# ruuda/robigo-luculenta

Hardware: AMD Instinct MI355X
Metric: Mrays/sec on built-in scene at 1920x1080 (higher is better)
Workload: dtype f32

## Files before the change

### robigo_luculenta_amd/csrc/rl_api.hip

```cpp
#include <hip/hip_runtime.h>
#include <sys/prctl.h>

#include <dlfcn.h>
#include <unistd.h>

#include <algorithm>
#include <chrono>
#include <condition_variable>
#include <cstdio>
#include <cstdlib>
#include <cstring>
#include <atomic>
#include <map>
#include <memory>
#include <mutex>
#include <new>
#include <string>
#include <thread>
#include <vector>

#include <rccl/rccl.h>

#include "../../include/robigo_luculenta.h"
#include "../../include/robigo_luculenta_debug.h"
// ... 174 lines not shown
    };
    return table[index];
}
size_t ring_t_bytes(const RlScene* scene) { return scene->lay.n_cluster_supers != 0u ? (size_t)(RL_TRACE_BLOCK / 64) * 512u : 0u; }
int stage_of(const RlScene* scene, int fetch, size_t scratch_bytes, size_t* bytes) {
    *bytes = 0;
    if (fetch != RL_FETCH_LDS) return RL_STAGE_NONE;
    const size_t all = (scene->staged_bytes + 511) & ~(size_t)511, tables = (scene->tables_bytes + 511) & ~(size_t)511;
    if (scene->lay.n_cluster_supers == 0u && all + scratch_bytes <= 160 * 1024) {
        *bytes = all;
        return RL_STAGE_ALL;
    }
    if (tables + scratch_bytes <= 160 * 1024) {
        *bytes = tables;
        return RL_STAGE_TABLES;
    }
    return RL_STAGE_NONE;
}

int fetch_check(int fetch) {
    if (fetch != RL_FETCH_LDS && fetch != RL_FETCH_GLOBAL) return fail(RL_E_INVALID, "unknown fetch mode");
    return RL_OK;
}
int path_range_check(uint64_t first_path, uint64_t n) {
    if (first_path + n < first_path || first_path + n == ~0ull) return fail(RL_E_INVALID, "path indices must stay below 2^64 - 1");
    return RL_OK;
}
int max_segments_resolve(uint32_t max_segments, uint32_t* resolved) {
    if (max_segments > RL_PATH_MAX_SEGMENTS_CAP) return fail(RL_E_INVALID, "max_segments exceeds RL_PATH_MAX_SEGMENTS_CAP = 65536");
    *resolved = max_segments == 0u ? RL_PATH_MAX_SEGMENTS : max_segments;
    return RL_OK;
}

int launch_trace(RlTraceUnit* u, const RlScene* scene, RlMappedPhoton* photons, RlPlotUnit* plot_unit, uint64_t seed,
                 uint32_t stream_id, uint64_t first_path, uint64_t n_paths) {
    if (n_paths == 0) return RL_OK;
    if (path_range_check(first_path, n_paths) != RL_OK) return RL_E_INVALID;
    float* plot = plot_unit ? plot_unit->xyz : nullptr;
    if (scene->device != u->device) return fail(RL_E_STATE, "scene and trace unit live on different devices");
    RlTraceJob job;
    job.width = u->width;
    job.height = u->height;
    job.aspect_ratio = (float)u->width / (float)u->height;
    job.stream = stream_id;
    job.seed = seed;
    job.first_path = first_path;
    job.n_paths = n_paths;
    job.grace_ticks = 0;
    job.reserved = 0;
    job.wm1 = (float)(int)u->width - 1.0f;
    job.hm1 = (float)(int)u->height - 1.0f;

    const size_t scratch_bytes = (RL_TRACE_BLOCK / 64) * sizeof(RlWaveScratch) + ring_t_bytes(scene);
    size_t blob_bytes = 0;
    const int stage = stage_of(scene, u->fetch, scratch_bytes, &blob_bytes);
    const bool fused = plot != nullptr;
    const bool cyl = scene->lay.prism_cylinders != 0u;
    auto kernel = trace_kernel_variant(stage, fused, false, cyl);
    const size_t dyn = scratch_bytes + blob_bytes;
    if (u->tuned_per_cu == 0 || u->tuned_dyn != dyn || u->tuned_kernel != (const void*)kernel) {
        RL_HIP(hipFuncSetAttribute((const void*)kernel, hipFuncAttributeMaxDynamicSharedMemorySize, 160 * 1024));
        int per_cu = 1;
        RL_HIP(hipOccupancyMaxActiveBlocksPerMultiprocessor(&per_cu, kernel, RL_TRACE_BLOCK, dyn));
        u->tuned_per_cu = per_cu < 1 ? 1 : per_cu;
        if (getenv("RL_DEBUG_LAUNCH")) fprintf(stderr, "rl: trace launch: %d workgroup(s) of %d threads per CU, %zu bytes of LDS each, stage %d\n", per_cu, RL_TRACE_BLOCK, dyn, stage);
        u->tuned_dyn = dyn;
        u->tuned_kernel = (const void*)kernel;
    }
    uint64_t blocks = (uint64_t)u->cu_count * (uint64_t)u->tuned_per_cu;
    const uint64_t needed = (n_paths + RL_TRACE_BLOCK - 1) / RL_TRACE_BLOCK;
// ... 2411 lines not shown
```

### robigo_luculenta_amd/csrc/rl_kernels.hip.h

```cpp
#pragma once
#include <hip/hip_runtime.h>

#include <cstddef>
#include <type_traits>

#include "rl_cie1931.h"
#include "rl_core.h"

#define RL_BLOCK 256
#ifndef RL_TRACE_BLOCK
#define RL_TRACE_BLOCK 1024
#endif
#ifndef RL_TRACE_WPS
#define RL_TRACE_WPS 4
#endif
#ifndef RL_TRACE_VGPRS
#define RL_TRACE_VGPRS (RL_TRACE_WPS == 4 ? 128 : 96)
#endif
#ifndef RL_TRACE_VGPRS_OPEN
#define RL_TRACE_VGPRS_OPEN (RL_TRACE_WPS == 4 ? 120 : 96)
#endif
#define RL_EMIT_MAX_AGE 8u
#define RL_CHUNK 256ull

// ... 158 lines not shown
    float lhs;
    asm("v_fma_f32 %0, %1, %2, %3" : "=v"(lhs) : "v"(x), "v"(y), "v"(cs));
    return lhs;
}
__device__ __forceinline__ bool rl_cull_pass(const RlCullRay& r, RlF4 b, float far) {
    const float dd = __builtin_fmaf(r.d.z, b.z, __builtin_fmaf(r.d.y, b.y, __builtin_fmaf(r.d.x, b.x, r.p)));
    const float cs = __builtin_fmaf(r.m.z, b.z, __builtin_fmaf(r.m.y, b.y, __builtin_fmaf(r.m.x, b.x, b.w)));
    const float x = __builtin_amdgcn_fmed3f(dd, 0.0f, far);
    return __builtin_fmaf(x, __builtin_fmaf(-2.0f, dd, x), cs) <= r.q;
}

__device__ __forceinline__ bool rl_cyl_pass(const RlCullRay& r, RlF4 c, RlF3 a) {
    const float cox = __builtin_fmaf(0.5f, r.m.x, c.x), coy = __builtin_fmaf(0.5f, r.m.y, c.y), coz = __builtin_fmaf(0.5f, r.m.z, c.z);
    const float crx = __builtin_fmaf(r.d.y, a.z, -(r.d.z * a.y)), cry = __builtin_fmaf(r.d.z, a.x, -(r.d.x * a.z)),
                crz = __builtin_fmaf(r.d.x, a.y, -(r.d.y * a.x));
    const float w = __builtin_fmaf(coz, crz, __builtin_fmaf(coy, cry, cox * crx));
    const float radius = __builtin_fmaf(4.0e-6f, fabsf(cox) + fabsf(coy) + fabsf(coz), c.w);
    const float cr2 = __builtin_fmaf(crz, crz, __builtin_fmaf(cry, cry, crx * crx));
    return !(w * w > radius * radius * cr2);
}

struct RlWaveScratch {
    unsigned long long key[64];
    uint32_t ring_a[128];
    uint32_t ring_b[128];
    uint32_t ring_s[128];
    float terms_d[64][4];
    float terms_m[64][4];
    float far[64];
    float stash[10][64];
    float emit[5][64];
};
static_assert(sizeof(RlWaveScratch) == 8192, "rl_scan_wave's ring addressing wants the wave's scratch 512-byte aligned");

typedef float RlV4 __attribute__((ext_vector_type(4)));
typedef __attribute__((address_space(3))) RlV4 RlLdsV4;
typedef __attribute__((address_space(3))) float RlLdsF;
template <bool PF = false>
__device__ __forceinline__ void rl_store_cull_ray(RlWaveScratch* ws, uint32_t lane, const RlCullRay& cr, float far) {
    ((RlLdsV4*)&ws->terms_d[0][0])[lane] = (RlV4){cr.d.x, cr.d.y, cr.d.z, cr.p};
    ((RlLdsV4*)&ws->terms_m[0][0])[lane] = (RlV4){cr.m.x, cr.m.y, cr.m.z, cr.q};
    ((RlLdsF*)&ws->far[0])[lane] = PF ? cr.len : far;
}
template <bool PF = false>
__device__ __forceinline__ void rl_fetch_cull_ray(RlWaveScratch* ws, uint32_t owner, RlCullRay& r, float& r_far) {
    const RlV4 a = ((const RlLdsV4*)&ws->terms_d[0][0])[owner], b = ((const RlLdsV4*)&ws->terms_m[0][0])[owner];
    r_far = ((const RlLdsF*)&ws->far[0])[owner];
    if (PF) r_far *= rl_u2f(((const RlLdsU32*)&ws->key[0])[2u * owner + 1u]);
    r.d = rl_f3(a.x, a.y, a.z);
    r.p = a.w;
    r.m = rl_f3(b.x, b.y, b.z);
    r.q = b.w;
    r.len = 0.0f;
}
__device__ __forceinline__ void rl_fetch_ray(RlWaveScratch* ws, uint32_t owner, RlF3 dir, RlF3& ro, RlF3& rd) {
    const RlV4 b = ((const RlLdsV4*)&ws->terms_m[0][0])[owner];
    rl_fetch3(owner, dir.x, dir.y, dir.z, rd.x, rd.y, rd.z);
    asm volatile("" : : "v"(b.w));
    ro = rl_f3(b.x * -0.5f, b.y * -0.5f, b.z * -0.5f);
}

struct RlOpenWg {
    uint32_t fin[RL_OPEN_CAP];
    uint32_t seg[RL_OPEN_CAP];
    uint32_t flushed_at;
    uint32_t poll[2];
    uint32_t pad;
};

template <bool CYL, bool SPLIT, bool UNROLL_S, bool HOIST_S, bool SPHERES_IN_LDS, bool TABLES_IN_LDS, bool SUPER, bool BOUNDED = false>
__device__ __forceinline__ RlHit rl_scan_wave(const RlSceneView& sv, const RlF4* cull, const RlF4* prism_cyl, uint32_t group_gc, uint32_t small_ordered, float sv_cull_cmax2,
                                              uint32_t n_cluster_groups, uint32_t n_prism_groups, uint32_t n_cluster_supers, uint32_t super_g, RlLdsU32* ring_t, RlF3 o, RlF3 dir,
                                              uint32_t idle_bit, RlWaveScratch* ws, uint32_t lane RL_TACC_PARAM, float t_bound = 1.0e12f) {
    constexpr bool PF = SUPER;
    RlLdsU64* keys = (RlLdsU64*)ws->key;
    RlLdsU32* ring_a = (RlLdsU32*)ws->ring_a;
    RlLdsU32* ring_b = (RlLdsU32*)ws->ring_b;
    RlLdsU32* ring_s = (RlLdsU32*)ws->ring_s;
    uint32_t a_lim = 64u, a_tail = 0, b_lim = 64u, b_tail = 0, s_lim = 64u, s_tail = 0;
    const uint32_t ws_addr = (uint32_t)(size_t)(RlLdsU32*)ws;
#define RL_RING_SLOT(RING, M, TAIL) \
    ((RlLdsU32*)(size_t)((ws_addr | (((rl_mbcnt(M) + (TAIL)) << 2) & 0x1fcu)) + (uint32_t)offsetof(RlWaveScratch, RING)))
#define RL_RING_PUSH(RING, COND, M, TAIL, ENTRY)                                                                        \
    {                                                                                                                   \
        uint32_t slot_;                                                                                                 \
                \
        asm volatile("s_mov_b64 exec, %6\n\ts_nop 0\n\tv_mbcnt_lo_u32_b32 %0, %1, 0\n\tv_mbcnt_hi_u32_b32 %0, %2, %0\n\t"         \
                     "v_add_lshl_u32 %0, %0, %3, 2\n\tv_and_or_b32 %0, %0, %4, %5\n\tds_write_b32 %0, %7 offset:%8\n\ts_mov_b64 exec, -1" \
                     : "=&v"(slot_)                                                                                     \
                     : "s"((uint32_t)(M)), "s"((uint32_t)((M) >> 32)), "s"(TAIL), "s"(ring_mask), "v"(ws_addr), "s"(M),  \
                       "v"(ENTRY), "n"(offsetof(RlWaveScratch, RING))                                                   \
                     : "memory");                                                                                       \
    }
#define RL_LE_PUSH(RING, LHS, RHS, TAIL, ENTRY)                                                                        \
    {                                                                                                                   \
        uint32_t slot_, n_;                                                                                             \
         \
        asm volatile("v_cmpx_le_f32_e32 vcc, %2, %3\n\ts_bcnt1_i32_b64 %1, vcc\n\ts_nop 0\n\t"                              \
                     "v_mbcnt_lo_u32_b32 %0, vcc_lo, 0\n\tv_mbcnt_hi_u32_b32 %0, vcc_hi, %0\n\t"                            \
                     "v_add_lshl_u32 %0, %0, %4, 2\n\tv_and_or_b32 %0, %0, %5, %6\n\tds_write_b32 %0, %7 offset:%8\n\t"     \
                     "s_mov_b64 exec, -1"                                                                               \
                     : "=&v"(slot_), "=&s"(n_)                                                                           \
                     : "v"(LHS), "v"(RHS), "s"(TAIL), "s"(ring_mask), "v"(ws_addr), "v"(ENTRY),                          \
// ... 91 lines not shown
            RL_FENCE;
            parab(b0, b1, b2);
            const RlF4 d0 = sv.planes[0], d1 = sv.planes[1];
            RL_FENCE;
            parab(c0, c1, c2);
            const RlF4 e0 = sv.planes[2], e1 = sv.planes[3];
            RL_FENCE;
            plane(d0, d1);
            const RlF4 f0 = sv.planes[4], f1 = sv.planes[5];
            RL_FENCE;
            plane(e0, e1);
            plane(f0, f1);
#undef RL_FENCE
        };
        if ((small_ordered & 2u) != 0u) six(std::integral_constant<bool, true>());
        else six(std::integral_constant<bool, false>());
    } else if ((small_ordered & 1u) != 0u) {
        RL_SMALL_PRIMITIVES(RL_NEARER_ORDERED, n_parabs, n_planes)
    } else {
        RL_SMALL_PRIMITIVES(rl_nearer, n_parabs, n_planes)
    }
#undef RL_NEARER_ORDERED
#undef RL_SMALL_PRIMITIVES
    keys[lane] = ((unsigned long long)rl_f2u(best.t) << 32) |
                 (unsigned long long)(best.obj == RL_HIT_NONE ? 0xffffffffu : (best.obj << 3));
    RL_T1(RL_ST_T_SMALL, t_small);
    if constexpr (BOUNDED) {
        if (best.obj != RL_HIT_NONE && best.t < t_bound) idle_bit = 0x80000000u;
        if (__builtin_amdgcn_ballot_w64(idle_bit == 0u) == 0) return best;
    }

    RlCullRay cr = rl_cull_ray(o, dir, sv_cull_cmax2, idle_bit != 0u);
    float far = best.t * cr.len;
    rl_store_cull_ray<PF>(ws, lane, cr, far);
#define RL_REFRESH_FAR()                                                                                \
    if (PF) {                                                                                           \
        far = rl_u2f(((const RlLdsU32*)keys)[2u * lane + 1u]) * cr.len;                                 \
         \
        if constexpr (BOUNDED) {                                                                        \
            if (rl_u2f(((const RlLdsU32*)keys)[2u * lane + 1u]) < t_bound) cr.q = -__builtin_inff();    \
        }                                                                                               \
    }

    auto process_spheres = [&](uint32_t count) {
        RL_STAT(RL_ST_B_ROUNDS, 1);
        RL_STAT(RL_ST_B_LANES, count);
        RL_T0(t_b);
        rl_wave_sync();
        const uint32_t e = ring_b[(b_lim - 64u + lane) & 127u];
        const uint32_t owner = e & 63u;
        const uint32_t pos = (SPHERES_IN_LDS || lane < count) ? e >> 6 : 0u;
        const RlF4 s = sph[pos];
        const float s_r2 = sv.sphere_r2[pos];
        const uint32_t s_obj = sv.sphere_obj[pos];
        RlF3 fo, fd;
        rl_fetch_ray(ws, owner, dir, fo, fd);
        asm volatile("" : : "v"(s.w));
        const float ox = fo.x, oy = fo.y, oz = fo.z, dx = fd.x, dy = fd.y, dz = fd.z;
        if (lane < count) {
            const float cox = s.x - ox, coy = s.y - oy, coz = s.z - oz;
            const float dd = dx * cox + dy * coy + dz * coz;
            const float c = (cox * cox + coy * coy + coz * coz) - s_r2;
            const float q = dd * dd - c;
            const float sq = rl_sqrtf(q, true);
            const float t1 = dd - sq;
            const float t2 = dd + sq;
            if ((q >= 0.0f) & (t1 > 0.0f) & (t1 < t2)) {
                __hip_atomic_fetch_min(keys + owner, ((unsigned long long)rl_f2u(t1) << 32) | (unsigned long long)(s_obj << 3),
                                       __ATOMIC_RELAXED, __HIP_MEMORY_SCOPE_WAVEFRONT);
            }
        }
        rl_wave_sync();
        RL_T1(RL_ST_T_B_ROUNDS, t_b);
    };

#define RL_SPHERE_REJECT(S, POS, OWNER, DISABLE_BIT, OX, OY, OZ, DX, DY, DZ)                        \
    {                                                                                               \
        const float cox = (S).x - (OX), coy = (S).y - (OY), coz = (S).z - (OZ);                     \
        const float dd = (DX) * cox + (DY) * coy + (DZ) * coz;                                      \
        const float c = (cox * cox + coy * coy + coz * coz) - (S).w;                                \
        const float q = dd * dd - c;                                                                \
        const bool cand = (int)(rl_f2u(q) | (rl_f2u(dd) - 1u) | (DISABLE_BIT)) >= 0;               \
        const uint64_t m = __builtin_amdgcn_ballot_w64(cand);                                       \
        if (m != 0) {                                                                               \
            RL_RING_PUSH(ring_b, cand, m, b_tail, ((POS) << 6) | (OWNER))               \
            b_tail += (uint32_t)__popcll(m);                                                        \
            if (RL_UNLIKELY(b_tail >= b_lim)) {                                                           \
                process_spheres(64u);                                                               \
                b_lim += 64u;                                                                      \
// ... 295 lines not shown
#undef RL_SPHERE_REJECT
    RL_T1(RL_ST_T_CLUSTER, t_cluster);
    RL_T0(t_tailflush);
    if (b_tail != b_lim - 64u) process_spheres(b_tail - (b_lim - 64u));
    b_lim = b_tail + 64u;
    RL_T1(RL_ST_T_TAIL, t_tailflush);
    RL_T0(t_prism);
    far = rl_u2f((uint32_t)(keys[lane] >> 32)) * cr.len;
    if (!PF) ((RlLdsF*)&ws->far[0])[lane] = far;
    if constexpr (BOUNDED) {
        const unsigned long long k_now = keys[lane];
        if (rl_u2f((uint32_t)(k_now >> 32)) < t_bound) idle_bit = 0x80000000u;
        if (__builtin_amdgcn_ballot_w64(idle_bit == 0u) == 0) {
            best.t = rl_u2f((uint32_t)(k_now >> 32));
            best.obj = (uint32_t)k_now == 0xffffffffu ? RL_HIT_NONE : (uint32_t)k_now >> 3;
            best.sub = (uint32_t)k_now == 0xffffffffu ? 0u : (uint32_t)k_now & 7u;
            return best;
        }
    }

    auto process_prisms = [&](uint32_t count) {
        RL_STAT(RL_ST_P_ROUNDS, 1);
        RL_STAT(RL_ST_P_LANES, count);
        RL_T0(t_p);
        rl_wave_sync();
        uint32_t e = ring_a[(a_lim - 64u + lane) & 127u];
        uint32_t owner = e & 63u;
        const uint32_t prism = e >> 6;
        const RlF4* pr = sv.prisms + __umul24((uint32_t)RL_PRISM_STRIDE, lane < count ? prism : 0u);
        constexpr bool PRE = HOIST_S && SPLIT;
        RlF4 pre_n = RlF4(), pre_off = RlF4();
        if (PRE) pre_n = pr[0], pre_off = pr[1];
        RlF3 ro, rd;
        rl_fetch_ray(ws, owner, dir, ro, rd);
        RlCand c;
        int status = rl_hex_prism_fast<HOIST_S && SPLIT, PRE>(pr, ro, rd, &c, pre_n, pre_off);
        if (lane >= count) status = RL_PRISM_MISS;
        if (__builtin_amdgcn_ballot_w64(status == RL_PRISM_UNSURE) != 0) {
            RL_STAT(RL_ST_P_SLOW, 1);
            c = rl_hex_prism(pr, ro, rd);
            status = ((lane < count) & (c.t >= 0.0f)) ? RL_PRISM_HIT : RL_PRISM_MISS;
            {
                asm volatile("" ::: "memory");
                const float keep_len = cr.len;
                rl_fetch_cull_ray<PF>(ws, lane, cr, far);
                cr.len = keep_len;
            }
            uint32_t again = a_lim - 64u;
            asm volatile("" : "+s"(again) : : "memory");
            e = ring_a[(again + lane) & 127u];
            owner = e & 63u;
            pr = sv.prisms + __umul24((uint32_t)RL_PRISM_STRIDE, lane < count ? (e >> 6) : 0u);
        }
        if (status == RL_PRISM_HIT) {
            const uint32_t obj = rl_f2u(pr[1].w);
            const unsigned long long k = ((unsigned long long)rl_f2u(c.t) << 32) | (unsigned long long)((obj << 3) | c.k);
            __hip_atomic_fetch_min(keys + owner, k, __ATOMIC_RELAXED, __HIP_MEMORY_SCOPE_WAVEFRONT);
        }
        rl_wave_sync();
        RL_T1(RL_ST_T_P_ROUNDS, t_p);
    };
    auto process_cylinders = [&](uint32_t count) {
        rl_wave_sync();
        const uint32_t e = ring_b[(b_lim - 64u + lane) & 127u];
        const uint32_t owner = e & 63u;
        const RlF4* cy = prism_cyl + 2u * (lane < count ? (e >> 6) : 0u);
        const RlF4 cy0 = cy[0], cy1 = cy[1];
// ... 171 lines not shown
#endif
    typedef __attribute__((address_space(3))) float RlLdsF32;
    RlLdsF32* stash = (RlLdsF32*)&ws->stash[0][0];

    uint64_t chunk_next = 0, chunk_end = 0;
    uint32_t stash_head = 0, stash_count = 0;
    uint64_t stash_path0 = 0;
    uint32_t stash_valid = 0;
    bool drained = false;
    bool active = false;
    uint64_t my_path = 0;
    uint32_t my_job = 0;
    uint32_t stash_job = 0;
    uint64_t stash_first = job.first_path;
    RlPath p;
    p.origin = rl_f3(0.0f, 0.0f, 0.0f);
    p.direction = rl_f3(0.0f, 0.0f, 0.0f);
    p.wavelength = 0.0f;
    p.intensity = 0.0f;
    p.continue_chance = 0.0f;
    p.sx = p.sy = 0.0f;
    p.ior = 1.0f;
    p.bounce = 0;
    uint32_t segments = 0, paths_done = 0;
    uint32_t known_local = 0;
    bool pend_me = false;
    bool pend_any = false;
    uint32_t emit_pend = 0;
    RlOpenWg* wgp = (RlOpenWg*)(scratch + RL_TRACE_BLOCK / 64);
    RlLdsU32* wg_fin = (RlLdsU32*)&wgp->fin[0];
    RlLdsU32* wg_seg = (RlLdsU32*)&wgp->seg[0];
    RlLdsU32* wg_flushed_at = (RlLdsU32*)&wgp->flushed_at;
    RlLdsU32* wg_poll = (RlLdsU32*)&wgp->poll[0];
    RlLdsF32* emit = (RlLdsF32*)&ws->emit[0][0];
    auto emit_put = [&](uint32_t row, uint32_t slot, float v) {
        emit[row * 64u + slot] = v;
    };
    auto emit_get = [&](uint32_t row, uint32_t slot) -> float {
        return emit[row * 64u + slot];
    };
    if (OPEN) {
        for (uint32_t i = threadIdx.x; i < sizeof(RlOpenWg) / 4; i += RL_TRACE_BLOCK) ((RlLdsU32*)wgp)[i] = 0;
        __syncthreads();
    }
    auto settle = [&]() {
        if (!pend_any && emit_pend == 0) return;
        asm volatile("s_waitcnt vmcnt(0) ; rl_settle: results acknowledged" ::: "memory");
        __builtin_amdgcn_fence(__ATOMIC_RELEASE, "workgroup");
        if (pend_me) __hip_atomic_fetch_add(wg_fin + my_job, 1u, __ATOMIC_RELAXED, __HIP_MEMORY_SCOPE_WORKGROUP);
        if (lane < emit_pend)
            __hip_atomic_fetch_add(wg_fin + (((RlLdsU32*)ws->ring_b)[lane] >> 24), 1u, __ATOMIC_RELAXED,
                                   __HIP_MEMORY_SCOPE_WORKGROUP);
        pend_me = false;
        pend_any = false;
        emit_pend = 0;
    };
    auto flush = [&](uint32_t gap) {
        const uint32_t now = (uint32_t)wall_clock64();
        uint32_t mine = gap == 0u ? 1u : 0u;
        if (lane == 0 && gap != 0u) {
            uint32_t at = *wg_flushed_at;
            if (now - at >= gap)
                mine = __hip_atomic_compare_exchange_strong(wg_flushed_at, &at, now | 1u, __ATOMIC_RELAXED, __ATOMIC_RELAXED,
                                                            __HIP_MEMORY_SCOPE_WORKGROUP) ? 1u : 0u;
        }
        if (__builtin_amdgcn_readfirstlane(mine) == 0u) return;
        for (uint32_t base_job = 0; base_job < known_local; base_job += 64u) {
// ... 6 lines not shown
            if (__builtin_amdgcn_ballot_w64((f | sg) != 0u) == 0) continue;
            if (sg != 0) __hip_atomic_fetch_add(&od->seg[jb], sg, __ATOMIC_RELAXED, __HIP_MEMORY_SCOPE_AGENT);
            __builtin_amdgcn_fence(__ATOMIC_RELEASE, "workgroup");
            if (f != 0) {
                const uint32_t before = __hip_atomic_fetch_add(&od->fin[jb], f, __ATOMIC_RELAXED, __HIP_MEMORY_SCOPE_AGENT);
                if (before + f == (uint32_t)od->jobs[jb].end) {
                    __hip_atomic_fetch_add(&od->completed, 1u, __ATOMIC_RELAXED, __HIP_MEMORY_SCOPE_AGENT);
                    const uint32_t total = __hip_atomic_load(&od->seg[jb], __ATOMIC_RELAXED, __HIP_MEMORY_SCOPE_AGENT);
                    __hip_atomic_store(&ctl->segs[jb], total, __ATOMIC_RELAXED, __HIP_MEMORY_SCOPE_SYSTEM);
                    __hip_atomic_store(&ctl->done[jb], 1u, __ATOMIC_RELEASE, __HIP_MEMORY_SCOPE_SYSTEM);
                }
            }
        }
    };
    uint32_t e_head = 0, e_tail = 0;
    uint32_t emit_age = 0;
#ifdef RL_STATS
    unsigned long long st[RL_ST_COUNT];
    for (int k = 0; k < RL_ST_COUNT; ++k) st[k] = 0;
#endif
    RL_T0(t_total);

    auto process_emitted = [&](uint32_t count) {
        RL_STAT(RL_ST_EMIT_BATCHES, 1);
        RL_STAT(RL_ST_EMIT_LANES, count);
        if (OPEN && emit_pend != 0) settle();
        rl_wave_sync();
        if (!FUSED) {
            uint32_t idx = 0, tagged = 0;
            float value = 0.0f;
            RlMappedPhoton* dst_base = photons;
            if (lane < count) {
                const uint32_t slot = (e_head + lane) & 63u;
                idx = rl_f2u(emit_get(0, slot));
                tagged = rl_f2u(emit_get(4, slot));
                if (OPEN) ((RlLdsU32*)ws->ring_b)[lane] = tagged;
                uint64_t first = job.first_path;
                if (OPEN) {
                    const RlJobEntry e = jobs[tagged >> 24];
                    first = e.first_path, dst_base = (RlMappedPhoton*)e.target;
                }
                const RlRngBlock b0 = rl_rng_block(job.seed, job.stream, first + idx, 0);
                RlMappedPhoton ph;
                ph.wavelength = rl_get_wavelength(b0.w[0]);
                ph.x = rl_get_bi_unit(b0.w[1]);
                ph.y = rl_get_bi_unit(b0.w[2]) / job.aspect_ratio;
                value = rl_emission(sv, emit_get(3, slot), ph.wavelength, OPEN ? (tagged & 0xffffffu) : tagged);
                ph.probability = value;
                if (OPEN) {
                    uint32_t* dst = (uint32_t*)&dst_base[idx];
                    __hip_atomic_store(dst + 0, rl_f2u(ph.x), __ATOMIC_RELAXED, __HIP_MEMORY_SCOPE_AGENT);
                    __hip_atomic_store(dst + 1, rl_f2u(ph.y), __ATOMIC_RELAXED, __HIP_MEMORY_SCOPE_AGENT);
                    __hip_atomic_store(dst + 2, rl_f2u(ph.probability), __ATOMIC_RELAXED, __HIP_MEMORY_SCOPE_AGENT);
                    __hip_atomic_store(dst + 3, rl_f2u(ph.wavelength), __ATOMIC_RELAXED, __HIP_MEMORY_SCOPE_AGENT);
                } else {
                    dst_base[idx] = ph;
                }
            }
        } else if (lane < count) {
            const uint32_t slot = (e_head + lane) & 63u;
            const float sx = emit_get(0, slot), sy = emit_get(1, slot), wavelength = emit_get(2, slot);
            const uint32_t tagged = rl_f2u(emit_get(4, slot));
            if (OPEN) ((RlLdsU32*)ws->ring_b)[lane] = tagged;
            float* target = plot;
            if (OPEN) target = (float*)jobs[tagged >> 24].target;
            const float value = rl_emission(sv, emit_get(3, slot), wavelength, OPEN ? (tagged & 0xffffffu) : tagged);
            if (value != 0.0f) {
                const RlF3 cie = rl_mul(rl_tristimulus(sv.cie, wavelength), value);
                uint32_t width = job.width, height = job.height;
                asm volatile("" : "+s"(width), "+s"(height));
                const RlSplat sp = rl_splat_weights(width, height, job.wm1, job.hm1, job.aspect_ratio, sx, sy);
#pragma unroll
                for (int k = 0; k < 4; ++k) {
                    float* px = target + 3ull * sp.idx[k];
                    unsafeAtomicAdd(px + 0, cie.x * sp.w[k]);
                    unsafeAtomicAdd(px + 1, cie.y * sp.w[k]);
                    unsafeAtomicAdd(px + 2, cie.z * sp.w[k]);
                }
            }
        }
        if (OPEN) emit_pend = count;
        rl_wave_sync();
    };

    for (;;) {
        if (OPEN) {
            settle();
            flush(3000u);
        }
        RL_T0(t_refill);
        auto refill = [&]() -> bool {
            if (drained) return false;
                uint32_t open_n = 0;
                if (OPEN) {
                    bool got = false;
                    for (;;) {
                        if (chunk_next < chunk_end) {
                            open_n = (uint32_t)jobs[stash_job].end;
                            got = true;
// ... 101 lines not shown
                    }
                    if (!got) return false;
                }
                if (!OPEN && chunk_next == chunk_end) {
                    const unsigned long long chunk =
                        job.n_paths >= (unsigned long long)gridDim.x * (RL_TRACE_BLOCK * 16ull) ? RL_CHUNK : 64ull;
                    unsigned long long b = 0;
                    if (lane == 0) b = atomicAdd(&queue[0], chunk);
                    const uint32_t lo = __builtin_amdgcn_readfirstlane((uint32_t)b);
                    const uint32_t hi = __builtin_amdgcn_readfirstlane((uint32_t)(b >> 32));
                    chunk_next = ((uint64_t)hi << 32) | lo;
                    chunk_end = chunk_next + chunk;
                }
                RL_STAT(RL_ST_REFILLS, 1);
                if (OPEN) stash_first = jobs[stash_job].first_path;
                const uint64_t limit = OPEN ? (uint64_t)open_n : job.n_paths;
                stash_path0 = stash_first + chunk_next;
                stash_valid = chunk_next >= limit ? 0u : (limit - chunk_next >= 64ull ? 64u : (uint32_t)(limit - chunk_next));
                chunk_next += 64;
                const bool valid = lane < stash_valid;
                const uint64_t path_index = stash_path0 + lane;
                RlPath fresh = p;
                RL_T0(t_cam);
                if (valid) rl_begin_path(sv, job.aspect_ratio, job.seed, job.stream, path_index, &fresh);
                RL_T1(RL_ST_T_CAMERA, t_cam);
                rl_wave_sync();
                stash[0 * 64 + lane] = fresh.origin.x;
                stash[1 * 64 + lane] = fresh.origin.y;
                stash[2 * 64 + lane] = fresh.origin.z;
                stash[3 * 64 + lane] = fresh.direction.x;
                stash[4 * 64 + lane] = fresh.direction.y;
                stash[5 * 64 + lane] = fresh.direction.z;
                stash[6 * 64 + lane] = fresh.wavelength;
                stash[7 * 64 + lane] = fresh.sx;
                stash[8 * 64 + lane] = fresh.sy;
                stash[9 * 64 + lane] = fresh.ior;
                rl_wave_sync();
                stash_head = 0;
                stash_count = 64;
                if (!OPEN && chunk_next >= job.n_paths) drained = true;
            return true;
        };
        auto hand_out = [&](const uint64_t need) -> bool {
            const uint32_t avail = stash_count - stash_head;
            const uint32_t rank = rl_mbcnt(need);
            const uint32_t slot = stash_head + rank;
            const bool take = !active & (rank < avail) & (slot < stash_valid);
            {
                const uint32_t sl = slot & 63u;
                const float s0 = stash[0 * 64 + sl], s1 = stash[1 * 64 + sl], s2 = stash[2 * 64 + sl], s3 = stash[3 * 64 + sl], s4 = stash[4 * 64 + sl];
                const float s5 = stash[5 * 64 + sl], s6 = stash[6 * 64 + sl], s7 = stash[7 * 64 + sl], s8 = stash[8 * 64 + sl], s9 = stash[9 * 64 + sl];
                my_path = take ? stash_path0 + slot : my_path;
                if (OPEN) my_job = take ? stash_job : my_job;
                p.origin = rl_f3(take ? s0 : p.origin.x, take ? s1 : p.origin.y, take ? s2 : p.origin.z);
                p.direction = rl_f3(take ? s3 : p.direction.x, take ? s4 : p.direction.y, take ? s5 : p.direction.z);
                p.wavelength = take ? s6 : p.wavelength;
                p.sx = take ? s7 : p.sx;
                p.sy = take ? s8 : p.sy;
                p.ior = take ? s9 : p.ior;
                p.intensity = take ? 1.0f : p.intensity;
                p.continue_chance = take ? 1.0f : p.continue_chance;
                p.bounce = take ? 0u : p.bounce;
                active = active | take;
            }
            const uint32_t wanted = (uint32_t)__popcll(need);
            stash_head += wanted < avail ? wanted : avail;
            return wanted <= avail;
        };
        {
            const uint64_t need = __builtin_amdgcn_ballot_w64(!active);
            if (need != 0) {
                bool served = false;
                if (RL_LIKELY(stash_count != stash_head)) served = hand_out(need);
                if (RL_UNLIKELY(!served)) {
                    if (refill()) hand_out(__builtin_amdgcn_ballot_w64(!active));
                }
            }
        }
        RL_T1(RL_ST_T_REFILL, t_refill);
        if (__builtin_amdgcn_ballot_w64(active) == 0) {
            if (!OPEN || drained) break;
            settle();
            if (e_tail != e_head) {
                process_emitted(e_tail - e_head);
                e_head = e_tail;
                settle();
            }
            flush(500u);
            for (int k = 0; k < 4; ++k) __builtin_amdgcn_s_sleep(127);
            continue;
        }
        constexpr bool FULL = !OPEN || (STAGE == RL_STAGE_ALL && (FUSED || !CYL));
        const RlHit hit = rl_scan_wave<CYL, FULL, STAGE != RL_STAGE_NONE && (!(FUSED && OPEN) || FULL), STAGE != RL_STAGE_NONE && (!(OPEN && (FUSED || STAGE == RL_STAGE_TABLES)) || FULL), STAGE == RL_STAGE_ALL, STAGE != RL_STAGE_NONE, STAGE != RL_STAGE_ALL>(sv, base + (lay.off_cull - tab0), CYL ? base + (lay.off_prism_cyl - tab0) : nullptr, lay.group_gc, lay.small_ordered, lay.cull_cmax2, lay.n_cluster_groups, lay.n_prism_groups,
                                       lay.n_cluster_supers, lay.super_g, ring_t, p.origin, p.direction, active ? 0u : 0x80000000u, ws, lane RL_TACC_ARG);
#ifdef RL_STATS
        {
            const uint32_t mk = (active && hit.obj != RL_HIT_NONE) ? rl_object_material(rl_f2u(sv.objects[hit.obj].w)) : 99u;
            const uint64_t m_act = __builtin_amdgcn_ballot_w64(active);
            const uint64_t m_void = __builtin_amdgcn_ballot_w64(active && hit.obj == RL_HIT_NONE);
            const uint64_t m_emit = __builtin_amdgcn_ballot_w64(mk == RL_MATERIAL_BLACK_BODY);
            const uint64_t m_grey = __builtin_amdgcn_ballot_w64(mk == RL_MATERIAL_DIFFUSE_GREY);
            const uint64_t m_col = __builtin_amdgcn_ballot_w64(mk == RL_MATERIAL_DIFFUSE_COLOURED);
            const uint64_t m_gls = __builtin_amdgcn_ballot_w64(mk == RL_MATERIAL_GLOSSY_MIRROR);
            const uint64_t m_glass = __builtin_amdgcn_ballot_w64(mk == RL_MATERIAL_SF10_GLASS);
            const uint64_t m_soap = __builtin_amdgcn_ballot_w64(mk == RL_MATERIAL_SOAP_BUBBLE);
            RL_STAT(RL_ST_ITER, 1);
            RL_STAT(RL_ST_SCAN_LANES, __popcll(m_act));
            RL_STAT(RL_ST_END_VOID, __popcll(m_void));
            RL_STAT(RL_ST_END_EMITTER, __popcll(m_emit));
            RL_STAT(RL_ST_SHADE_DIFFUSE, __popcll(m_grey | m_col | m_gls));
            RL_STAT(RL_ST_SHADE_GLASS, __popcll(m_glass));
            RL_STAT(RL_ST_SHADE_SOAP, __popcll(m_soap));
            RL_STAT(RL_ST_ANY_DIFFUSE, (m_grey | m_col | m_gls) != 0);
            RL_STAT(RL_ST_ANY_GLASS, m_glass != 0);
            RL_STAT(RL_ST_ANY_SOAP, m_soap != 0);
            RL_STAT(RL_ST_ANY_COLOURED, m_col != 0);
            RL_STAT(RL_ST_ANY_GLOSSY, m_gls != 0);
        }
#endif
        RL_T0(t_shade);
        bool ended_on_emitter = false, ended_now = false;
        uint32_t emit_obj = 0, emit_idx = 0;
        if (active) {
            segments += 1;
            float value;
            uint32_t emitter = 0;
            const int status = rl_bounce(sv, job.seed, job.stream, my_path, &p, hit, &value, &emitter);
            if (status != RL_PATH_CONTINUES) {
                active = false;
                p.direction = rl_f3(0.0f, 0.0f, 0.0f);
                paths_done += 1;
                ended_on_emitter = status == RL_PATH_ENDED_ON_EMITTER;
                emit_obj = OPEN ? (emitter | (my_job << 24)) : emitter;
                if (!FUSED && !ended_on_emitter) {
                    RlMappedPhoton ph;
                    ph.x = p.sx;
                    ph.y = p.sy;
                    ph.probability = value;
                    ph.wavelength = p.wavelength;
                    if (OPEN) {
                        const RlJobEntry e = jobs[my_job];
                        uint32_t* dst = (uint32_t*)&((RlMappedPhoton*)e.target)[my_path - e.first_path];
                        __hip_atomic_store(dst + 0, rl_f2u(ph.x), __ATOMIC_RELAXED, __HIP_MEMORY_SCOPE_AGENT);
                        __hip_atomic_store(dst + 1, rl_f2u(ph.y), __ATOMIC_RELAXED, __HIP_MEMORY_SCOPE_AGENT);
                        __hip_atomic_store(dst + 2, rl_f2u(ph.probability), __ATOMIC_RELAXED, __HIP_MEMORY_SCOPE_AGENT);
                        __hip_atomic_store(dst + 3, rl_f2u(ph.wavelength), __ATOMIC_RELAXED, __HIP_MEMORY_SCOPE_AGENT);
                    } else {
                        photons[my_path - job.first_path] = ph;
                    }
                }
                if (!FUSED && ended_on_emitter) emit_idx = (uint32_t)(my_path - (OPEN ? jobs[my_job].first_path : job.first_path));
                if (OPEN) {
                    ended_now = true;
                    __hip_atomic_fetch_add(wg_seg + my_job, p.bounce + ((hit.obj == RL_HIT_NONE || status == RL_PATH_ENDED_ON_EMITTER) ? 1u : 0u),
                                           __ATOMIC_RELAXED, __HIP_MEMORY_SCOPE_WORKGROUP);
                }
            }
        }
        if (OPEN) {
            pend_me = ended_now && !ended_on_emitter;
            pend_any = __builtin_amdgcn_ballot_w64(pend_me) != 0;
            ended_now = false;
        }
        RL_T1(RL_ST_T_SHADE, t_shade);
        RL_T0(t_emit);
        {
            const uint64_t m = __builtin_amdgcn_ballot_w64(ended_on_emitter);
            if (m != 0) {
                const uint32_t n_new = (uint32_t)__popcll(m);
                if (RL_UNLIKELY(e_tail - e_head + n_new > 64u)) {
                    process_emitted(e_tail - e_head);
                    e_head = e_tail;
                }
                if (ended_on_emitter) {
                    const uint32_t slot = rl_mbcnt_from(m, e_tail) & 63u;
                    if (FUSED) {
                        emit_put(0, slot, p.sx);
                        emit_put(1, slot, p.sy);
                        emit_put(2, slot, p.wavelength);
                    } else {
                        emit_put(0, slot, rl_u2f(emit_idx));
                    }
                    emit_put(3, slot, p.intensity);
                    emit_put(4, slot, rl_u2f(emit_obj));
                    ended_on_emitter = false;
                }
                e_tail += n_new;
                if (RL_UNLIKELY(e_tail - e_head == 64u)) {
                    process_emitted(64u);
                    e_head += 64u;
                }
            }
            if (OPEN && !FUSED) {
                emit_age = e_tail != e_head ? emit_age + 1u : 0u;
                if (RL_UNLIKELY(emit_age >= RL_EMIT_MAX_AGE)) {
                    process_emitted(e_tail - e_head);
                    e_head = e_tail;
                    emit_age = 0;
                }
            }
        }
        RL_T1(RL_ST_T_EMIT, t_emit);
    }
    if (e_tail != e_head) process_emitted(e_tail - e_head);
    if (OPEN) {
        settle();
        flush(0u);
    }
    RL_T1(RL_ST_T_TOTAL, t_total);
#ifdef RL_STATS
    if (lane == 0)
        for (int k = 0; k < RL_ST_COUNT; ++k) atomicAdd(&rl_stat_counters[k], st[k]);
#endif
    uint32_t s = segments, d = paths_done;
#pragma unroll
    for (int off = 32; off > 0; off >>= 1) {
        s += __shfl_down(s, off);
// ... 268 lines not shown
```

Measured before the change: 22490.

## Cache ray directions in LDS and recompute fused emitter sample coords from RNG

In the fused kernel, the wave scratch gets a new layout that stores each lane's ray direction as a float4 in LDS. Primitive tests now read the direction from there instead of doing cross-lane fetches. Emitter records and the path stash stop carrying sx/sy/wavelength; the fused emit path regenerates them from the RNG block keyed by path index, which frees LDS rows for the direction array. It also splits trace launches above 2^31 paths. This trades cross-lane permutes and stash traffic for extra RNG recomputation at emission.

```diff
diff --git a/robigo_luculenta_amd/csrc/rl_api.hip b/robigo_luculenta_amd/csrc/rl_api.hip
--- a/robigo_luculenta_amd/csrc/rl_api.hip
+++ b/robigo_luculenta_amd/csrc/rl_api.hip
@@ -230,10 +230,18 @@
     return RL_OK;
 }
 
+#define RL_LAUNCH_MAX_PATHS (1ull << 31)
+
 int launch_trace(RlTraceUnit* u, const RlScene* scene, RlMappedPhoton* photons, RlPlotUnit* plot_unit, uint64_t seed,
                  uint32_t stream_id, uint64_t first_path, uint64_t n_paths) {
     if (n_paths == 0) return RL_OK;
     if (path_range_check(first_path, n_paths) != RL_OK) return RL_E_INVALID;
+    while (n_paths > RL_LAUNCH_MAX_PATHS) {
+        const int rc = launch_trace(u, scene, photons, plot_unit, seed, stream_id, first_path, RL_LAUNCH_MAX_PATHS);
+        if (rc != RL_OK) return rc;
+        first_path += RL_LAUNCH_MAX_PATHS, n_paths -= RL_LAUNCH_MAX_PATHS;
+        if (photons) photons += RL_LAUNCH_MAX_PATHS;
+    }
     float* plot = plot_unit ? plot_unit->xyz : nullptr;
     if (scene->device != u->device) return fail(RL_E_STATE, "scene and trace unit live on different devices");
     RlTraceJob job;
diff --git a/robigo_luculenta_amd/csrc/rl_kernels.hip.h b/robigo_luculenta_amd/csrc/rl_kernels.hip.h
--- a/robigo_luculenta_amd/csrc/rl_kernels.hip.h
+++ b/robigo_luculenta_amd/csrc/rl_kernels.hip.h
@@ -214,15 +214,27 @@
     float emit[5][64];
 };
 static_assert(sizeof(RlWaveScratch) == 8192, "rl_scan_wave's ring addressing wants the wave's scratch 512-byte aligned");
+struct RlWaveScratchFused {
+    unsigned long long key[64];
+    uint32_t ring_a[128], ring_b[128], ring_s[128];
+    float terms_d[64][4], terms_m[64][4], far[64];
+    float stash[8][64];
+    float emit[3][64];
+    float dir[64][4];
+};
+static_assert(sizeof(RlWaveScratchFused) == sizeof(RlWaveScratch), "one scratch size for every kernel: the host sizes the launches' LDS by it");
+static_assert(offsetof(RlWaveScratchFused, far) == offsetof(RlWaveScratch, far) && offsetof(RlWaveScratchFused, stash) == offsetof(RlWaveScratch, stash),
+              "the scan's part of the scratch is the same in both layouts");
 
 typedef float RlV4 __attribute__((ext_vector_type(4)));
 typedef __attribute__((address_space(3))) RlV4 RlLdsV4;
 typedef __attribute__((address_space(3))) float RlLdsF;
-template <bool PF = false>
-__device__ __forceinline__ void rl_store_cull_ray(RlWaveScratch* ws, uint32_t lane, const RlCullRay& cr, float far) {
+template <bool PF = false, bool DIRS = false>
+__device__ __forceinline__ void rl_store_cull_ray(RlWaveScratch* ws, uint32_t lane, const RlCullRay& cr, float far, RlF3 dir) {
     ((RlLdsV4*)&ws->terms_d[0][0])[lane] = (RlV4){cr.d.x, cr.d.y, cr.d.z, cr.p};
     ((RlLdsV4*)&ws->terms_m[0][0])[lane] = (RlV4){cr.m.x, cr.m.y, cr.m.z, cr.q};
     ((RlLdsF*)&ws->far[0])[lane] = PF ? cr.len : far;
+    if (DIRS) ((RlLdsV4*)&((RlWaveScratchFused*)ws)->dir[0][0])[lane] = (RlV4){dir.x, dir.y, dir.z, dir.z};
 }
 template <bool PF = false>
 __device__ __forceinline__ void rl_fetch_cull_ray(RlWaveScratch* ws, uint32_t owner, RlCullRay& r, float& r_far) {
@@ -235,10 +247,17 @@
     r.q = b.w;
     r.len = 0.0f;
 }
+template <bool DIRS = false>
 __device__ __forceinline__ void rl_fetch_ray(RlWaveScratch* ws, uint32_t owner, RlF3 dir, RlF3& ro, RlF3& rd) {
-    const RlV4 b = ((const RlLdsV4*)&ws->terms_m[0][0])[owner];
-    rl_fetch3(owner, dir.x, dir.y, dir.z, rd.x, rd.y, rd.z);
-    asm volatile("" : : "v"(b.w));
+    RlV4 b = ((const RlLdsV4*)&ws->terms_m[0][0])[owner];
+    if (DIRS) {
+        RlV4 d = ((const RlLdsV4*)&((RlWaveScratchFused*)ws)->dir[0][0])[owner];
+        asm volatile("" : "+v"(b), "+v"(d) : : "memory");
+        rd = rl_f3(d.x, d.y, d.z);
+    } else {
+        rl_fetch3(owner, dir.x, dir.y, dir.z, rd.x, rd.y, rd.z);
+        asm volatile("" : : "v"(b.w));
+    }
     ro = rl_f3(b.x * -0.5f, b.y * -0.5f, b.z * -0.5f);
 }
 
@@ -250,7 +269,7 @@
     uint32_t pad;
 };
 
-template <bool CYL, bool SPLIT, bool UNROLL_S, bool HOIST_S, bool SPHERES_IN_LDS, bool TABLES_IN_LDS, bool SUPER, bool BOUNDED = false>
+template <bool CYL, bool SPLIT, bool UNROLL_S, bool HOIST_S, bool SPHERES_IN_LDS, bool TABLES_IN_LDS, bool SUPER, bool BOUNDED = false, bool DIRS = false>
 __device__ __forceinline__ RlHit rl_scan_wave(const RlSceneView& sv, const RlF4* cull, const RlF4* prism_cyl, uint32_t group_gc, uint32_t small_ordered, float sv_cull_cmax2,
                                               uint32_t n_cluster_groups, uint32_t n_prism_groups, uint32_t n_cluster_supers, uint32_t super_g, RlLdsU32* ring_t, RlF3 o, RlF3 dir,
                                               uint32_t idle_bit, RlWaveScratch* ws, uint32_t lane RL_TACC_PARAM, float t_bound = 1.0e12f) {
@@ -408,7 +427,7 @@
 
     RlCullRay cr = rl_cull_ray(o, dir, sv_cull_cmax2, idle_bit != 0u);
     float far = best.t * cr.len;
-    rl_store_cull_ray<PF>(ws, lane, cr, far);
+    rl_store_cull_ray<PF, DIRS>(ws, lane, cr, far, dir);
 #define RL_REFRESH_FAR()                                                                                \
     if (PF) {                                                                                           \
         far = rl_u2f(((const RlLdsU32*)keys)[2u * lane + 1u]) * cr.len;                                 \
@@ -430,7 +449,7 @@
         const float s_r2 = sv.sphere_r2[pos];
         const uint32_t s_obj = sv.sphere_obj[pos];
         RlF3 fo, fd;
-        rl_fetch_ray(ws, owner, dir, fo, fd);
+        rl_fetch_ray<DIRS>(ws, owner, dir, fo, fd);
         asm volatile("" : : "v"(s.w));
         const float ox = fo.x, oy = fo.y, oz = fo.z, dx = fd.x, dy = fd.y, dz = fd.z;
         if (lane < count) {
@@ -792,7 +811,7 @@
         RlF4 pre_n = RlF4(), pre_off = RlF4();
         if (PRE) pre_n = pr[0], pre_off = pr[1];
         RlF3 ro, rd;
-        rl_fetch_ray(ws, owner, dir, ro, rd);
+        rl_fetch_ray<DIRS>(ws, owner, dir, ro, rd);
         RlCand c;
         int status = rl_hex_prism_fast<HOIST_S && SPLIT, PRE>(pr, ro, rd, &c, pre_n, pre_off);
         if (lane >= count) status = RL_PRISM_MISS;
@@ -1030,7 +1049,9 @@
     RlLdsU32* wg_seg = (RlLdsU32*)&wgp->seg[0];
     RlLdsU32* wg_flushed_at = (RlLdsU32*)&wgp->flushed_at;
     RlLdsU32* wg_poll = (RlLdsU32*)&wgp->poll[0];
-    RlLdsF32* emit = (RlLdsF32*)&ws->emit[0][0];
+    RlLdsF32* emit = FUSED ? (RlLdsF32*)&((RlWaveScratchFused*)ws)->emit[0][0] : (RlLdsF32*)&ws->emit[0][0];
+    constexpr uint32_t E_IDX = 0u, E_INTENSITY = FUSED ? 1u : 3u, E_OBJ = FUSED ? 2u : 4u;
+    constexpr uint32_t STASH_IOR = FUSED ? 7u : 9u;
     auto emit_put = [&](uint32_t row, uint32_t slot, float v) {
         emit[row * 64u + slot] = v;
     };
@@ -1103,8 +1124,8 @@
             RlMappedPhoton* dst_base = photons;
             if (lane < count) {
                 const uint32_t slot = (e_head + lane) & 63u;
-                idx = rl_f2u(emit_get(0, slot));
-                tagged = rl_f2u(emit_get(4, slot));
+                idx = rl_f2u(emit_get(E_IDX, slot));
+                tagged = rl_f2u(emit_get(E_OBJ, slot));
                 if (OPEN) ((RlLdsU32*)ws->ring_b)[lane] = tagged;
                 uint64_t first = job.first_path;
                 if (OPEN) {
@@ -1116,7 +1137,7 @@
                 ph.wavelength = rl_get_wavelength(b0.w[0]);
                 ph.x = rl_get_bi_unit(b0.w[1]);
                 ph.y = rl_get_bi_unit(b0.w[2]) / job.aspect_ratio;
-                value = rl_emission(sv, emit_get(3, slot), ph.wavelength, OPEN ? (tagged & 0xffffffu) : tagged);
+                value = rl_emission(sv, emit_get(E_INTENSITY, slot), ph.wavelength, OPEN ? (tagged & 0xffffffu) : tagged);
                 ph.probability = value;
                 if (OPEN) {
                     uint32_t* dst = (uint32_t*)&dst_base[idx];
@@ -1130,12 +1151,21 @@
             }
         } else if (lane < count) {
             const uint32_t slot = (e_head + lane) & 63u;
-            const float sx = emit_get(0, slot), sy = emit_get(1, slot), wavelength = emit_get(2, slot);
-            const uint32_t tagged = rl_f2u(emit_get(4, slot));
+            const uint32_t idx = rl_f2u(emit_get(E_IDX, slot));
+            const uint32_t tagged = rl_f2u(emit_get(E_OBJ, slot));
             if (OPEN) ((RlLdsU32*)ws->ring_b)[lane] = tagged;
             float* target = plot;
-            if (OPEN) target = (float*)jobs[tagged >> 24].target;
-            const float value = rl_emission(sv, emit_get(3, slot), wavelength, OPEN ? (tagged & 0xffffffu) : tagged);
+            uint64_t first = job.first_path;
+            if (OPEN) {
+                const RlJobEntry e = jobs[tagged >> 24];
+                first = e.first_path, target = (float*)e.target;
+            }
+            const RlRngBlock b0 = rl_rng_block(job.seed, job.stream, first + idx, 0);
+            const float wavelength = rl_get_wavelength(b0.w[0]);
+            const float sx = rl_get_bi_unit(b0.w[1]);
+            const float sy = rl_get_bi_unit(b0.w[2]) / job.aspect_ratio;
+            __builtin_amdgcn_sched_barrier(0);
+            const float value = rl_emission(sv, emit_get(E_INTENSITY, slot), wavelength, OPEN ? (tagged & 0xffffffu) : tagged);
             if (value != 0.0f) {
                 const RlF3 cie = rl_mul(rl_tristimulus(sv.cie, wavelength), value);
                 uint32_t width = job.width, height = job.height;
@@ -1303,9 +1333,11 @@
                 stash[4 * 64 + lane] = fresh.direction.y;
                 stash[5 * 64 + lane] = fresh.direction.z;
                 stash[6 * 64 + lane] = fresh.wavelength;
-                stash[7 * 64 + lane] = fresh.sx;
-                stash[8 * 64 + lane] = fresh.sy;
-                stash[9 * 64 + lane] = fresh.ior;
+                if (!FUSED) {
+                    stash[7 * 64 + lane] = fresh.sx;
+                    stash[8 * 64 + lane] = fresh.sy;
+                }
+                stash[STASH_IOR * 64 + lane] = fresh.ior;
                 rl_wave_sync();
                 stash_head = 0;
                 stash_count = 64;
@@ -1320,14 +1352,16 @@
             {
                 const uint32_t sl = slot & 63u;
                 const float s0 = stash[0 * 64 + sl], s1 = stash[1 * 64 + sl], s2 = stash[2 * 64 + sl], s3 = stash[3 * 64 + sl], s4 = stash[4 * 64 + sl];
-                const float s5 = stash[5 * 64 + sl], s6 = stash[6 * 64 + sl], s7 = stash[7 * 64 + sl], s8 = stash[8 * 64 + sl], s9 = stash[9 * 64 + sl];
+                const float s5 = stash[5 * 64 + sl], s6 = stash[6 * 64 + sl], s7 = FUSED ? 0.0f : stash[7 * 64 + sl], s8 = FUSED ? 0.0f : stash[8 * 64 + sl], s9 = stash[STASH_IOR * 64 + sl];
                 my_path = take ? stash_path0 + slot : my_path;
                 if (OPEN) my_job = take ? stash_job : my_job;
                 p.origin = rl_f3(take ? s0 : p.origin.x, take ? s1 : p.origin.y, take ? s2 : p.origin.z);
                 p.direction = rl_f3(take ? s3 : p.direction.x, take ? s4 : p.direction.y, take ? s5 : p.direction.z);
                 p.wavelength = take ? s6 : p.wavelength;
-                p.sx = take ? s7 : p.sx;
-                p.sy = take ? s8 : p.sy;
+                if (!FUSED) {
+                    p.sx = take ? s7 : p.sx;
+                    p.sy = take ? s8 : p.sy;
+                }
                 p.ior = take ? s9 : p.ior;
                 p.intensity = take ? 1.0f : p.intensity;
                 p.continue_chance = take ? 1.0f : p.continue_chance;
@@ -1362,7 +1396,7 @@
             continue;
         }
         constexpr bool FULL = !OPEN || (STAGE == RL_STAGE_ALL && (FUSED || !CYL));
-        const RlHit hit = rl_scan_wave<CYL, FULL, STAGE != RL_STAGE_NONE && (!(FUSED && OPEN) || FULL), STAGE != RL_STAGE_NONE && (!(OPEN && (FUSED || STAGE == RL_STAGE_TABLES)) || FULL), STAGE == RL_STAGE_ALL, STAGE != RL_STAGE_NONE, STAGE != RL_STAGE_ALL>(sv, base + (lay.off_cull - tab0), CYL ? base + (lay.off_prism_cyl - tab0) : nullptr, lay.group_gc, lay.small_ordered, lay.cull_cmax2, lay.n_cluster_groups, lay.n_prism_groups,
+        const RlHit hit = rl_scan_wave<CYL, FULL, STAGE != RL_STAGE_NONE && (!(FUSED && OPEN) || FULL), STAGE != RL_STAGE_NONE && (!(OPEN && (FUSED || STAGE == RL_STAGE_TABLES)) || FULL), STAGE == RL_STAGE_ALL, STAGE != RL_STAGE_NONE, STAGE != RL_STAGE_ALL, false, FUSED>(sv, base + (lay.off_cull - tab0), CYL ? base + (lay.off_prism_cyl - tab0) : nullptr, lay.group_gc, lay.small_ordered, lay.cull_cmax2, lay.n_cluster_groups, lay.n_prism_groups,
                                        lay.n_cluster_supers, lay.super_g, ring_t, p.origin, p.direction, active ? 0u : 0x80000000u, ws, lane RL_TACC_ARG);
 #ifdef RL_STATS
         {
@@ -1420,7 +1454,7 @@
                         photons[my_path - job.first_path] = ph;
                     }
                 }
-                if (!FUSED && ended_on_emitter) emit_idx = (uint32_t)(my_path - (OPEN ? jobs[my_job].first_path : job.first_path));
+                if (ended_on_emitter) emit_idx = (uint32_t)(my_path - (OPEN ? jobs[my_job].first_path : job.first_path));
                 if (OPEN) {
                     ended_now = true;
                     __hip_atomic_fetch_add(wg_seg + my_job, p.bounce + ((hit.obj == RL_HIT_NONE || status == RL_PATH_ENDED_ON_EMITTER) ? 1u : 0u),
@@ -1445,15 +1479,9 @@
                 }
                 if (ended_on_emitter) {
                     const uint32_t slot = rl_mbcnt_from(m, e_tail) & 63u;
-                    if (FUSED) {
-                        emit_put(0, slot, p.sx);
-                        emit_put(1, slot, p.sy);
-                        emit_put(2, slot, p.wavelength);
-                    } else {
-                        emit_put(0, slot, rl_u2f(emit_idx));
-                    }
-                    emit_put(3, slot, p.intensity);
-                    emit_put(4, slot, rl_u2f(emit_obj));
+                    emit_put(E_IDX, slot, rl_u2f(emit_idx));
+                    emit_put(E_INTENSITY, slot, p.intensity);
+                    emit_put(E_OBJ, slot, rl_u2f(emit_obj));
                     ended_on_emitter = false;
                 }
                 e_tail += n_new;
```

After: 22590 (median of 6 runs). No clear change (+0.4%).
